# facebookresearch/FlowDec

Hardware: AMD Instinct MI355X
Metric: 48 kHz audio-seconds/sec (RTF) for FlowDec-75m @ 6 ODE steps (higher is better)
Workload: dtype bf16; 1 GPU; flowdec_75m enhance(): global batch=8 x 2 s clips @48 kHz (8 per GPU), 6-step euler (NFE 6), T_pad=256 frames, inputs resident in HBM, initial noise drawn inside the timed call, output waveforms all-gathered; global_batch=8, nfe=6, parallelism=batch-shard x1, hipgraph=True, conv_algo=auto

## Files before the change

flowdec_amd/_lib.py:

```python
import ctypes as C
import os

import torch

_HERE = os.path.dirname(os.path.abspath(__file__))
LIB_PATH = os.environ.get("FLOWDEC_HIP_LIB") or os.path.join(_HERE, "libflowdec_hip.so")

FD_F32, FD_BF16 = 0, 1
FD_WINOGRAD = 0x100
FD_WINOGRAD4 = 0x80000
FD_TILE_REVERSED = 0x100000
FD_WINOGRAD44 = 0x200000
FD_WINOGRAD_LOWRES = 0x200
FD_WINOGRAD_AUTO = 0x400
FD_LOW_LATENCY = 0x800
FD_BF16_OPERANDS = 0x10000
FD_NO_SIDE_STREAM = 0x40000
FD_EBUSY = -5
FD_BF16X3_OPERANDS = 0x20000
FD_TILE = {0: 0, 32: 0x1000, 64: 0x2000, 128: 0x3000, "64c": 0x4000, "32c": 0x5000, "duo": 0x6000, "persist": 0x7000}
CONV_KERNELS = ("DIRECT", "DIRECT_MIXED", "DIRECT_SPLIT", "WINO", "WINO4", "WINO4F", "WINO44F", "HEAD", "HEADF")
FIR_FAMILIES = ("UP", "DOWN", "DOWN_MARCH")
SOLVERS = {"euler": 0, "midpoint": 1, "heun2": 2, "heun2_eulerlast": 3}
ADAPTIVE_SOLVERS = {"dopri5": 0, "tsit5": 1}
# ... 62 lines not shown
    "fd_gn_silu_apply": (c_int, [_P, _P, _P, c_int, c_ll, c_int, c_int, _P]),
    "fd_op_pack_input": (c_int, [_P, _P, _P, c_int, c_int, c_int, c_int, _P]),
    "fd_op_combine": (c_int, [_P, _P, _P, _P, _P, _P, c_int, c_int, c_int, c_int, c_int, _P]),
    "fd_op_output_update": (c_int, [_P, _P, _P, _P, c_float, _P, _P, c_int, c_int, c_int, c_int, c_int, _P]),
    "fd_op_score_update": (c_int, [_P, _P, _P, c_float, _P, c_float, c_float, _P, _P, c_int, c_float, _P, c_int, c_int, c_int, c_int, c_int, _P]),
    "fd_op_init_state": (c_int, [_P, _P, _P, _P, c_int, _P, c_int, c_float, _P, c_int, c_int, c_int, _P]),
    "fd_op_caxpy": (c_int, [_P, _P, _P, c_int, c_float, _P, c_int, c_int, c_int, _P]),
    "fd_op_ode_lincomb": (c_int, [_P, c_float, c_float, C.POINTER(_P), C.POINTER(c_float), c_int, _P, c_ll, _P]),
    "fd_op_ode_lincomb_clips": (c_int, [_P, c_float, _P, C.POINTER(_P), C.POINTER(c_float), c_int, _P, c_int, c_ll, _P]),
    "fd_op_ode_scaled_sq": (c_int, [_P, _P, _P, _P, c_float, c_float, _P, c_int, c_ll, _P]),
    "fd_op_ode_scaled_sq_clips": (c_int, [_P, _P, _P, _P, c_float, c_float, _P, c_int, c_int, c_ll, _P]),
    "fd_op_ode_commit_clips": (c_int, [_P, _P, _P, _P, _P, _P, _P, c_int, c_ll, _P]),
    "fd_resblock_workspace_bytes": (c_size_t, [C.POINTER(FdResblockDesc), c_int, c_int, c_int, c_int]),
    "fd_resblock": (c_int, [C.POINTER(FdResblockDesc), _P, _P, _P, c_int, c_int, c_int, c_int, _P, c_size_t, _P]),
    "fd_attn_block_workspace_bytes": (c_size_t, [C.POINTER(FdAttnDesc), c_int, c_int, c_int, c_int]),
    "fd_attn_block": (c_int, [C.POINTER(FdAttnDesc), _P, _P, _P, c_int, c_int, c_int, c_int, _P, c_size_t, _P]),
    "fd_gn_finalize": (c_int, [_P, c_int, c_int, c_int, _P, c_int, c_int, c_int, _P, _P, _P, c_int, c_int, c_ll, c_float, _P]),
    "fd_conv_packed_bytes": (c_ll, [c_int] * 7),
    "fd_conv_pack_weights": (c_int, [_P, _P, _P, c_int, c_int, c_int, c_int, c_int, c_int, c_int, _P]),
    "fd_conv_cout_pad": (c_int, [c_int]),
    "fd_conv_stats_tiles": (c_int, [c_int, c_int]),
    "fd_conv2d": (c_int, [_P, c_int, _P, c_int, _P, _P, c_int, _P, c_int, _P, _P, c_int, _P, c_float, _P, c_int, _P,
                          c_int, c_int, c_int, c_int, c_int, _P]),
    "fd_conv_kernel_counts": (c_int, [C.POINTER(c_ll), c_int]),
    "fd_time_embedding": (c_int, [_P, c_int, _P, c_int, _P, _P, _P, _P, _P, _P]),
    "fd_temb_bias": (c_int, [_P, c_int, c_int, _P, _P, _P, c_int, _P, _P]),
    "fd_stft_workspace_bytes": (c_size_t, [c_int] * 4),
    "fd_stft_plan_create": (c_int, [c_int, c_int, C.POINTER(c_void_p)]),
    "fd_stft_plan_destroy": (None, [_P]),
    "fd_stft_compress": (c_int, [_P, _P, c_int, c_int, c_float, c_float, c_int, _P, _P, c_int, _P, c_size_t, _P]),
    "fd_decompress_istft": (c_int, [_P, _P, c_int, c_int, c_int, c_float, c_float, _P, _P, c_int, _P, c_size_t, _P]),
    "fd_stft_compress_ragged": (c_int, [_P, _P, _P, c_int, c_int, c_float, c_float, c_int, _P, _P, c_int, _P, c_size_t, _P]),
    "fd_decompress_istft_ragged": (c_int, [_P, _P, _P, c_int, c_int, c_int, c_float, c_float, _P, _P, c_int, _P, c_size_t, _P]),
    "fd_compress_spec": (c_int, [_P, _P, c_ll, c_float, c_float, c_int, _P]),
    "fd_stft_tables": (c_int, [c_int, c_int, _P, _P, _P]),
    "fd_stft_gemm_variant": (c_int, [c_int] * 3),
    "fd_stft_gemm_f32": (c_int, [_P, _P, _P, c_int, c_int, c_int, _P]),
    "fd_istft_envelope_ok": (c_int, [c_int] * 4),
    "fd_num_frames": (c_int, [c_int, c_int]),
    "fd_padded_frames": (c_int, [c_int]),
    "fd_model_create": (c_int, [C.POINTER(FdModelConfig), C.POINTER(_P)]),
    "fd_model_create_ex": (c_int, [C.POINTER(FdModelConfig), C.POINTER(FdModelArch), C.POINTER(_P)]),
    "fd_model_destroy": (None, [_P]),
    "fd_model_num_params": (c_int, [_P]),
    "fd_model_param_info": (c_int, [_P, c_int, C.POINTER(C.c_char_p), C.POINTER(c_int), C.POINTER(c_int * 4)]),
    "fd_model_set_param": (c_int, [_P, C.c_char_p, _P, c_ll]),
# ... 147 lines not shown
```

flowdec_amd/build.py:

```python
import os
import subprocess
import sys
from concurrent.futures import ThreadPoolExecutor

HERE = os.path.dirname(os.path.abspath(__file__))
CSRC = os.path.join(HERE, "csrc")
INC = os.path.join(os.path.dirname(HERE), "include")
LIB = os.path.join(HERE, "libflowdec_hip.so")
SOURCES = ["api.hip", "calib.hip", "conv_mfma.hip", "conv_wino.hip", "conv_wino4.hip", "conv_wino4f.hip", "conv_wino44f.hip", "conv_head.hip", "conv_headf.hip", "elementwise.hip", "ops_api.hip", "stft.hip", "metrics.hip", "estimate.hip", "loss.hip", "model.hip", "solve.hip", "enhance.hip", "attn.hip", "ndac.hip", "ndac_mfma.hip", "stream.hip", "resample.hip", "stoi.hip", "specdist.hip", "xcorr.hip"]
FLAGS = ["--offload-arch=gfx950", "-O3", "-std=c++17", "-fPIC", "-fno-slp-vectorize", "-I" + INC, "-I" + CSRC, "-Wno-unused-result"]


def _hipcc():
    for c in (os.environ.get("HIPCC"), "/opt/rocm/bin/hipcc", "hipcc"):
        if c and (os.path.isabs(c) and os.path.exists(c) or not os.path.isabs(c)):
            return c
    return "hipcc"


def needs_build():
    if not os.path.exists(LIB):
        return True
    t = os.path.getmtime(LIB)
    deps = [os.path.join(CSRC, f) for f in os.listdir(CSRC)] + [os.path.join(INC, "flowdec_hip.h"), os.path.abspath(__file__)]
    return any(os.path.getmtime(d) > t for d in deps)


def check_wino4_isa(hipcc=None, extra=()):
    import tempfile
    if os.environ.get("FLOWDEC_SKIP_ISA_CHECK", "") not in ("", "0"):
        print("flowdec_amd.build: FLOWDEC_SKIP_ISA_CHECK set -- conv_wino4.hip ISA properties NOT verified", file=sys.stderr)
        return False
# ... 56 lines not shown
```

flowdec_amd/csrc/conv_common.h:

```cpp
#pragma once
#include "common.h"
#include "internal.h"

#ifdef FD_TIMING2
#define FD_T2(...) __VA_ARGS__
#else
#define FD_T2(...)
#endif

namespace fdconv {

typedef unsigned int u32x4 __attribute__((ext_vector_type(4)));

constexpr int ROWB = 80;
constexpr int WROWB = 64;
constexpr int PITCH = 24;

struct Seg {
  const void* src;
  int C;
  int aff_off;
  int taps;
};

// ... 39 lines not shown
int fd_wino4_launch(fdconv::ConvArgs a, hipStream_t st);
int fd_wino4_init_attributes();
bool fd_wino4_supported(int Cout, int C0, int C1, int S0, int S1, int ksize);
bool fd_wino4_shape_ok(int H, int W);

long long fd_wino4f_packed_bytes(int Cout, int C0, int C1, int S0, int S1);
int fd_wino4f_pack_weights(const float* w, const float* w_sc, void* packed, int Cout, int C0, int C1, int S0, int S1, hipStream_t st);
int fd_wino4f_launch(fdconv::ConvArgs a, hipStream_t st);
int fd_wino4f_init_attributes();
bool fd_wino4f_supported(int Cout, int C0, int C1, int S0, int S1, int ksize);
bool fd_wino4f_shape_ok(int H, int W);

long long fd_wino44f_packed_bytes(int Cout, int C0, int C1, int S0, int S1);
int fd_wino44f_pack_weights(const float* w, const float* w_sc, void* packed, int Cout, int C0, int C1, int S0, int S1, hipStream_t st);
int fd_wino44f_launch(fdconv::ConvArgs a, hipStream_t st);
int fd_wino44f_init_attributes();
bool fd_wino44f_supported(int Cout, int C0, int C1, int S0, int S1, int ksize);
bool fd_wino44f_shape_ok(int H, int W);

bool fd_head_supported(const fdconv::ConvArgs& a, int ksize, int dtype);
int fd_head_launch(fdconv::ConvArgs a, hipStream_t st);
int fd_head_init_attributes();

bool fd_headf_supported(const fdconv::ConvArgs& a, int ksize, int dtype);
int fd_headf_launch(fdconv::ConvArgs a, hipStream_t st);
int fd_headf_init_attributes();
```

flowdec_amd/csrc/conv_mfma.hip:

```cpp
#include <string.h>

#include <atomic>
#include <mutex>
#include <type_traits>

#include "conv_common.h"

namespace {

using namespace fdconv;
typedef float f32x2 __attribute__((ext_vector_type(2)));

template <typename T>
struct Math;
template <>
struct Math<bf16> {
  static constexpr int EPS = 8;
  __device__ static __forceinline__ void mma(f32x16& acc, const u32x4& wf, const u32x4& pf) {
    acc = __builtin_amdgcn_mfma_f32_32x32x16_bf16(__builtin_bit_cast(bf16x8, wf), __builtin_bit_cast(bf16x8, pf), acc, 0, 0, 0);
  }
};
template <>
struct Math<float> {
  static constexpr int EPS = 4;
// ... 1161 lines not shown
  a.affine = affine; a.affC = C0 + C1;
  a.w = packed_w; a.w_bytes = fd_conv_packed_bytes(Cout, C0, C1, ksize, S0, S1, dtype | (wino ? FD_WINOGRAD : 0) | (wino4 ? FD_WINOGRAD4 : 0) | (wino44 ? FD_WINOGRAD44 : 0) | (mixed ? FD_BF16_OPERANDS : 0) | (split ? FD_BF16X3_OPERANDS : 0));
  a.bias = bias; a.bias_rows = bias_rows; a.skip = skip; a.scale = scale; a.out = out; a.Cout = Cout; a.CoutPad = cout_pad(Cout);
  a.stats = stats; a.B = B; a.H = H; a.W = W; a.reversed = reversed ? 1 : 0;
  FD_T2(a.dbg = g_dbg;)
  FD_REQUIRE(a.w_bytes < (1ll << 31), "fd_conv2d: packed weights exceed 2 GiB");
  FD_REQUIRE(affine == nullptr || (C0 + C1) * 8 <= AFF_BYTES, "fd_conv2d: at most %d activated input channels", AFF_BYTES / 8);
  if (wino44) {
    FD_REQUIRE(fd_wino44f_supported(Cout, C0, C1, S0, S1, ksize) && fd_wino44f_shape_ok(H, W),
               "fd_conv2d: FD_F32 | FD_WINOGRAD44 needs ksize 3, Cout %% 128 == 0, channel counts %% 8 == 0, H %% 16 == W %% 16 == 0");
    return counted(FD_CONV_KERNEL_WINO44F, fd_wino44f_launch(a, fd_stream(stream)));
  }
  if (wino4f) return counted(FD_CONV_KERNEL_WINO4F, fd_wino4f_launch(a, fd_stream(stream)));
  if (wino4) return counted(FD_CONV_KERNEL_WINO4, fd_wino4_launch(a, fd_stream(stream)));
  if (wino) return counted(FD_CONV_KERNEL_WINO, fd_wino_launch(a, fd_stream(stream)));
  if (mixed) return counted(FD_CONV_KERNEL_DIRECT_MIXED, dispatch_conv_mixed(a, fd_stream(stream)));
  if (split) return counted(FD_CONV_KERNEL_DIRECT_SPLIT, dispatch_conv_split(a, fd_stream(stream)));
  if (bn_hint == 0 && fd_head_supported(a, ksize, dtype)) return counted(FD_CONV_KERNEL_HEAD, fd_head_launch(a, fd_stream(stream)));
  if (bn_hint == 0 && tile == 0 && fd_headf_supported(a, ksize, dtype)) return counted(FD_CONV_KERNEL_HEADF, fd_headf_launch(a, fd_stream(stream)));
  if (dtype == FD_BF16)
    return counted(FD_CONV_KERNEL_DIRECT, dispatch_conv<bf16>(a, fd_stream(stream), bn_hint, tile == FD_TILE_BN64_CHUNK || tile == FD_TILE_BN32_CHUNK, tile == FD_TILE_PERSIST));
  return counted(FD_CONV_KERNEL_DIRECT, dispatch_conv<float>(a, fd_stream(stream), bn_hint, false));
}
```

flowdec_amd/csrc/internal.h:

```cpp
#pragma once
#include "common.h"

struct fd_temb_job {
  const float* dense_w;
  const float* dense_b;
  const float* conv_b;
  float* out;
  int Cout;
};

struct fd_noise_src {
  const float* ptr = nullptr;
  const unsigned long long* seeds = nullptr;
  int draw = 0;
  const int* frame0 = nullptr;
};

struct fd_edge_args {
  const void* x = nullptr;
  const void* y = nullptr;
  const float* w = nullptr;
  const float* bias = nullptr;
  void* out = nullptr;
  const void* base = nullptr;
// ... 5 lines not shown
  float cb = 1.f, cy = 0.f, cz = 0.f;
  int B = 0, H = 0, W = 0, Cout = 0;
  int ks = 1;
};

int fd_time_embedding_impl(const float* t, float t_imm, int nt, const float* gfp_w, int nf, const float* w1, const float* b1,
                           const float* w2, const float* b2, float* temb, hipStream_t st);
int fd_temb_bias_batched(const fd_temb_job* jobs_dev, int njobs, const float* temb, int nt, int temb_dim, hipStream_t st);
int fd_edge_op(int which, const fd_edge_args& a, int dtype, hipStream_t st);
int fd_init_state(const float* Y, const fd_noise_src& noise, const double* sigma_dev, int sigma_n, float sigma_fac, float* x0, int B,
                  int F, int T, hipStream_t st);
int fd_combine_tiles(int H, int W);
int fd_ode_lincomb(const float* x, float cx, float dt, const float* const* k, const float* c, int nk, float* dst, long long n, hipStream_t st);
int fd_ode_scaled_sq(const float* p, const float* q, const float* r, const float* s, float atol, float rtol, double* partial, int nblocks,
                     long long n, hipStream_t st);
int fd_ode_lincomb_clips(const float* x, float cx, const float* dt_dev, const float* const* k, const float* c, int nk, float* dst, int B, long long n,
                         hipStream_t st);
int fd_ode_scaled_sq_clips(const float* p, const float* q, const float* r, const float* s, float atol, float rtol, double* partial, int nblocks, int B,
                           long long n, hipStream_t st);
int fd_ode_commit_clips(const int* accept, const int* ckpt, const float* x_new, const float* k6, float* x, float* k0, float* traj, int B, long long n,
                        hipStream_t st);
int fd_caxpy(const float* a, const fd_noise_src& q, float cq, float* dst, int B, int F, int T, hipStream_t st);
int fd_conv_init_attributes();
int fd_stft_forward(fd_stft_plan* p, const float* y, const int* lens, int B, int L, float alpha, float beta, int normalize, float* normfac,
                    float* Y, int T_pad, void* ws, size_t ws_bytes, hipStream_t st, const float* normfac_in = nullptr);
int fd_stft_inverse(fd_stft_plan* p, const float* X, const int* lens, int B, int T, int T_pad, float alpha, float beta, const float* normfac,
                    float* y, int L, void* ws, size_t ws_bytes, hipStream_t st);
size_t fd_stft_ws_bytes(int B, int L, int n_fft, int hop);
void fd_stft_plan_dims(const fd_stft_plan* p, int* n_fft, int* hop, int* n_freq, int* kpad);
int fd_stft_kpad(int n_fft);
int fd_stft_raw_spectrum(fd_stft_plan* p, const float* y, const int* lens, int B, int L, float* frames, float* spec, hipStream_t st);
void fd_resample_plan_dims(const fd_resample_plan* p, int* o, int* n, int* width, int* K);
bool fd_ndac_mfma_supported(int Ci, int Co, int K, int stride, int dil, int transposed);
void fd_ndac_mfma_pack(const float* w_ci_k_co, int Ci, int Co, int K, int stride, int transposed, void* dst);
int fd_ndac_mfma_conv(const float* x, const void* wp, const float* bias, const float* res, float* out, float* out_act, const float* alpha_out, int B,
                      int Ci, int T, int Co, int K, int stride, int pad, int dil, int transposed, hipStream_t st);
void fd_ndac_weight_ci_k_co(const float* w, int Ci, int Co, int K, int transposed, float* dst);
size_t fd_attn_qkv_bytes(int B, int N, int C);
int fd_attn_stats_tiles(int H, int W);
int fd_attn_launch(const void* x, const float* affine, const fd_attn_desc& d, float* qkv, void* out, float* stats, int B, int N, int dtype,
                   hipStream_t st);
```

flowdec_amd/csrc/model.hip:

```cpp
#include <string>
#include <vector>

#include "arena.h"
#include "model_internal.h"

using namespace fdm;

namespace {

struct Tens {
  size_t off = (size_t)-1;
  int C = 0, H = 0, W = 0;
  size_t sums = (size_t)-1;
  int tiles = 0, stride = 0;
};

int gn_groups(int C) { return (C / 4 < 32) ? C / 4 : 32; }

void build_structure(fd_model* m) {
  const fd_model_config& c = m->cfg;
  const int nf = c.nf, R = c.num_levels, nrb = c.num_res_blocks, nch = 4;
  auto& mods = m->mods;
  auto& P = m->params;
  mods.clear(); P.clear();
// ... 70 lines not shown
  FD_HIP(hipMemcpy(d, it->second.data(), sizeof(float) * it->second.size(), hipMemcpyHostToDevice));
  m->dev_allocs.push_back(d);
  m->dev_f32[name] = d;
  *out = d;
  return FD_OK;
}

int pack_conv(fd_model* m, const std::string& name, int Cout, int C0, int C1, const std::string& sc_name, int S0, int S1, int algo,
              const void** out, hipStream_t st) {
  float *src = nullptr, *sc = nullptr;
  FD_TRY(upload_f32(m, name, &src));
  if (!sc_name.empty()) FD_TRY(upload_f32(m, sc_name, &sc));
  void* dst = nullptr;
  const int wdtype = m->dt | algo | m->opflag;
  const long long bytes = fd_conv_packed_bytes(Cout, C0, C1, 3, S0, S1, wdtype);
  FD_REQUIRE(bytes > 0, "internal: no packing for conv '%s'", name.c_str());
  FD_HIP(hipMalloc(&dst, (size_t)bytes));
  m->dev_allocs.push_back(dst);
  FD_TRY(fd_conv_pack_weights(src, sc, dst, Cout, C0, C1, 3, S0, S1, wdtype, st));
  *out = dst;
  return FD_OK;
}

int pack_rb_conv(fd_model* m, int level, const std::string& name, int Cout, int C0, int C1, const std::string& sc_name, int S0, int S1,
                 ConvW* w, hipStream_t st) {
  auto fits = [&](int algo) { return fd_conv_packed_bytes(Cout, C0, C1, 3, S0, S1, m->dt | algo) > 0; };
  auto pack = [&](int algo, const void** out) { return pack_conv(m, name, Cout, C0, C1, sc_name, S0, S1, algo, out, st); };
  const bool f23_only = m->sched == CS_WINOGRAD || (m->sched == CS_WINOGRAD_LOWRES && level >= 2);
  if (f23_only && fits(FD_WINOGRAD)) return pack(FD_WINOGRAD, &w->f23);
  const bool by_size = m->sched == CS_AUTO || m->sched == CS_LATENCY;
  if (by_size && fits(FD_WINOGRAD)) FD_TRY(pack(FD_WINOGRAD, &w->f23));
  if (by_size && fits(FD_WINOGRAD4)) FD_TRY(pack(FD_WINOGRAD4, &w->f43));
  if (m->sched == CS_AUTO_F32 && fits(FD_WINOGRAD44)) FD_TRY(pack(FD_WINOGRAD44, &w->f44));
  return pack(0, &w->direct);
}

struct ConvPick { const void* w; int flags; };
ConvPick pick_conv(ConvSchedule s, const ConvW& w, int px_tiles, bool whole_tiles, int cin, int cout, bool shortcut) {
  const bool autosel = s == CS_AUTO, latency = s == CS_LATENCY;
  if (s == CS_AUTO_F32 && w.f44 && whole_tiles) return {w.f44, FD_WINOGRAD44};
  if (latency && px_tiles <= 24 && cout >= 64) return {w.direct, FD_TILE_BN32_CHUNK};
  if (autosel && px_tiles <= 16 && cout >= 64) return {w.direct, FD_TILE_BN64_CHUNK};
  if ((autosel || latency) && w.f23 && !shortcut && px_tiles <= (latency ? 128 : 96)) return {w.f23, FD_WINOGRAD};
  if ((autosel || (latency && px_tiles > 128)) && w.f43 && whole_tiles && cin >= 64) return {w.f43, FD_WINOGRAD4};
  if (latency && px_tiles <= 128 && cout >= 256 && cout % 128 == 0) return {w.direct, FD_TILE_BN128};
  return w.direct ? ConvPick{w.direct, 0} : ConvPick{w.f23, FD_WINOGRAD};
// ... 77 lines not shown
    int flags = pick.flags;
    if (flags == FD_WINOGRAD4 && !dry && (w4_launches++ & 1) != 0) flags |= FD_TILE_REVERSED;
    if (want_stats) {
      out.tiles = fd_conv_stats_tiles(out.H, out.W);
      out.stride = fd_conv_cout_pad(out.C);
      out.sums = arena.alloc(sizeof(float) * 2 * (size_t)B * out.tiles * out.stride);
    }
    if (dry) return FD_OK;
    const bool prof = m && m->profiling;
    auto launch = [&]() {
      return fd_conv2d(ptr(a.off), a.C, b ? ptr(b->off) : nullptr, b ? b->C : 0, aff == (size_t)-1 ? nullptr : (const float*)ptr(aff),
                       s0 ? ptr(s0->off) : nullptr, s0 ? s0->C : 0, s1 ? ptr(s1->off) : nullptr, s1 ? s1->C : 0, pick.w, bias, bias_rows,
                       skip ? ptr(skip->off) : nullptr, scale, ptr(out.off), out.C, want_stats ? (float*)ptr(out.sums) : nullptr, B,
                       out.H, out.W, ks, dt | flags | (m ? m->opflag : 0), st);
    };
    const int rc = prof ? timed(m->ev, m->ev_used, launch) : launch();
    if (prof) {
      const double csc = (s0 ? s0->C : 0) + (s1 ? s1->C : 0);
      m->prof_flops += 2.0 * B * out.H * out.W * (double)out.C * (cin * ks * ks + csc);
      const double exec = (flags & FD_WINOGRAD44) ? 0.25 : (flags & FD_WINOGRAD4) ? 0.5 : (flags & FD_WINOGRAD) ? 2.0 / 3.0 : 1.0;
      m->prof_flops_exec += 2.0 * B * out.H * out.W * (double)out.C * (cin * ks * ks * exec + csc);
      m->prof_bytes += (double)B * out.H * out.W * esz * (cin + csc + (skip ? out.C : 0) + out.C) + (double)esz * out.C * (cin * ks * ks + csc);
    }
    return rc;
  }

  int fir(const void* x, const float* aff, void* o_raw, void* o_act, int H, int W, int C, int dir) {
    const bool prof = m && m->profiling;
    auto launch = [&]() { return fd_fir_resample(x, aff, o_raw, o_act, B, H, W, C, dir, dt, st); };
    const int rc = prof ? timed(m->ev_fir, m->ev_fir_used, launch) : launch();
    if (prof) {
      const double in = (double)B * H * W * C * esz, out1 = dir > 0 ? 4.0 * in : 0.25 * in;
      m->prof_fir_bytes += in + out1 * ((o_raw ? 1 : 0) + (o_act ? 1 : 0));
    }
    return rc;
  }

  int resblock(const Mod& md, Tens& x0, Tens* x1, int nt, Tens& out, bool out_given = false) {
    const float rs2 = 0.70710678118654752440f;
    size_t aff0;
    FD_TRY(gn_affine(x0, x1, md.gn0_g, md.gn0_b, &aff0));
    const int H = x0.H, W = x0.W;
    const int OH = md.up ? 2 * H : (md.down ? H / 2 : H), OW = md.up ? 2 * W : (md.down ? W / 2 : W);
    Tens h1 = talloc(md.cout, OH, OW);
    Tens xr, hr;
    if (md.up || md.down) {
// ... 110 lines not shown
      }
      FD_TRY(resblock(mods[mi++], a1, nullptr, nt, a2));
      tfree(a1);
      h = a2;
    }
    Tens pyramid; bool have_pyr = false;
    for (int lvl = R - 1; lvl >= 0; --lvl) {
      for (int b = 0; b < nrb + 1; ++b) {
        Tens sk = hs.back(); hs.pop_back();
        Tens o;
        FD_TRY(resblock(mods[mi++], h, &sk, nt, o));
        tfree(h); tfree(sk);
        h = o;
      }
      const Mod& gn = mods[mi++];
      const Mod& head = mods[mi++];
      if (side) FD_TRY(fork());
      size_t aff;
      FD_TRY(gn_affine(h, nullptr, gn.gn0_g, gn.gn0_b, &aff));
      Tens pnew = talloc(4, h.H, h.W);
      if (have_pyr) {
        Tens pu = talloc(4, h.H, h.W);
        if (!dry) FD_TRY(fir(ptr(pyramid.off), nullptr, ptr(pu.off), nullptr, pyramid.H, pyramid.W, 4, +1));
        FD_TRY(conv(h, nullptr, aff, nullptr, nullptr, head.conv0, head.b_f32, 1, &pu, 1.f, pnew, false));
        release_later(pu.off, side); release_later(pyramid.off, side);
        pu.off = pyramid.off = (size_t)-1;
      } else {
        FD_TRY(conv(h, nullptr, aff, nullptr, nullptr, head.conv0, head.b_f32, 1, nullptr, 1.f, pnew, false));
      }
      release_later(aff, side);
      pyramid = pnew; have_pyr = true;
      if (side) back();
      if (lvl != 0) {
        Tens o;
        FD_TRY(resblock(mods[mi++], h, nullptr, nt, o));
        if (side) FD_TRY(join());
        tfree(h);
        h = o;
      } else if (side) {
        FD_TRY(join());
      }
    }
    tfree(h);
    if (!hs.empty() || mi != mods.size()) return fd_set_error(FD_ESTATE, "internal: module walk mismatch");
    if (!dry) {
      fd_edge_args a; a.x = ptr(pyramid.off); a.w = m->wo; a.base = os.base; a.kold = os.kold; a.coef = os.coef; a.out = os.dst; a.ksave = os.ksave;
      a.B = B; a.H = F; a.W = T; a.ks = m->arch.output_ksize;
      if (os.score) { a.y = os.yv; a.z = os.z; a.cb = os.cb; a.cy = os.cy; a.cz = os.cz; }
      FD_TRY(fd_edge_op(os.score ? 4 : 3, a, dt, st));
    }
    tfree(pyramid);
// ... 185 lines not shown
      case M_ATTN: {
        FD_TRY(upload_f32(m, p + "GroupNorm_0.weight", &md.gn0_g)); FD_TRY(upload_f32(m, p + "GroupNorm_0.bias", &md.gn0_b));
        const int Cc = md.cout;
        std::vector<float>& wq = m->host[p + "qkv.W"];
        std::vector<float>& bq = m->host[p + "qkv.b"];
        wq.assign((size_t)Cc * 3 * Cc, 0.f); bq.assign((size_t)3 * Cc, 0.f);
        for (int k = 0; k < 3; ++k) {
          const std::vector<float>& w = m->host[p + "NIN_" + std::to_string(k) + ".W"];
          const std::vector<float>& bb = m->host[p + "NIN_" + std::to_string(k) + ".b"];
          for (int r = 0; r < Cc; ++r)
            for (int c = 0; c < Cc; ++c) wq[(size_t)r * 3 * Cc + k * Cc + c] = w[(size_t)r * Cc + c];
          for (int c = 0; c < Cc; ++c) bq[(size_t)k * Cc + c] = bb[c];
        }
        FD_TRY(upload_f32(m, p + "qkv.W", &md.w_qkv)); FD_TRY(upload_f32(m, p + "qkv.b", &md.b_qkv));
        FD_TRY(upload_f32(m, p + "NIN_3.W", &md.w_f32)); FD_TRY(upload_f32(m, p + "NIN_3.b", &md.b_f32));
        break;
      }
      case M_GN:
        FD_TRY(upload_f32(m, p + "weight", &md.gn0_g));
        FD_TRY(upload_f32(m, p + "bias", &md.gn0_b));
        break;
      case M_CONV_HEAD:
        FD_TRY(pack_conv(m, p + "weight", md.cout, md.cin, 0, "", 0, 0, 0, &md.conv0.direct, st));
        FD_TRY(upload_f32(m, p + "bias", &md.b_f32));
        break;
      case M_RB: {
        FD_TRY(upload_f32(m, p + "GroupNorm_0.weight", &md.gn0_g)); FD_TRY(upload_f32(m, p + "GroupNorm_0.bias", &md.gn0_b));
        FD_TRY(upload_f32(m, p + "GroupNorm_1.weight", &md.gn1_g)); FD_TRY(upload_f32(m, p + "GroupNorm_1.bias", &md.gn1_b));
        FD_TRY(pack_rb_conv(m, md.level, p + "Conv_0.weight", md.cout, md.c0, md.c1, "", 0, 0, &md.conv0, st));
        FD_TRY(pack_rb_conv(m, md.level, p + "Conv_1.weight", md.cout, md.cout, 0, md.has_c2 ? p + "Conv_2.weight" : std::string(),
                            md.has_c2 ? md.c0 : 0, md.has_c2 ? md.c1 : 0, &md.conv1, st));
        if (md.has_c2) {
          std::vector<float>& b1 = m->host[p + "Conv_1.bias"];
          const std::vector<float>& b2 = m->host[p + "Conv_2.bias"];
          for (size_t i = 0; i < b1.size(); ++i) b1[i] += b2[i];
        }
        FD_TRY(upload_f32(m, p + "Conv_1.bias", &md.b1));
        fd_temb_job j{};
        FD_TRY(upload_f32(m, p + "Dense_0.weight", &tmp)); j.dense_w = tmp;
        FD_TRY(upload_f32(m, p + "Dense_0.bias", &tmp)); j.dense_b = tmp;
        FD_TRY(upload_f32(m, p + "Conv_0.bias", &tmp)); j.conv_b = tmp;
        md.bias0_eff = bias_pool + bias_off; bias_off += (size_t)fd_model::MAX_NT * md.cout;
        j.out = md.bias0_eff; j.Cout = md.cout;
        jobs.push_back(j);
        break;
      }
// ... 151 lines not shown
```

flowdec_amd/csrc/model_internal.h:

```cpp
#pragma once
#include <atomic>
#include <map>
#include <set>
#include <string>
#include <tuple>
#include <vector>

#include "common.h"
#include "internal.h"

namespace fdm {

enum ModKind { M_GFP, M_LINEAR, M_CONV_IN, M_RB, M_COMBINE, M_GN, M_CONV_HEAD, M_ATTN };

enum ConvSchedule { CS_DIRECT, CS_WINOGRAD, CS_WINOGRAD_LOWRES, CS_AUTO, CS_LATENCY, CS_AUTO_F32 };

struct ConvW { const void *direct = nullptr, *f23 = nullptr, *f43 = nullptr, *f44 = nullptr; };

struct Mod {
  ModKind kind;
  int idx;
  int cin = 0, cout = 0;
  int c0 = 0, c1 = 0;
  bool up = false, down = false, has_c2 = false;
  int level = 0;
  ConvW conv0, conv1;
  float *gn0_g = nullptr, *gn0_b = nullptr, *gn1_g = nullptr, *gn1_b = nullptr;
  float* b1 = nullptr;
  float* bias0_eff = nullptr;
  float *w_f32 = nullptr, *b_f32 = nullptr;
  float *w_qkv = nullptr, *b_qkv = nullptr;
};

struct ParamInfo {
  std::string name;
  std::vector<int> shape;
  long long numel() const { long long n = 1; for (int s : shape) n *= s; return n; }
};

struct GraphKey {
// ... 122 lines not shown
```

flowdec_amd/ops.py:

```python
import math

import torch

from . import _lib as L


def _nhwc(x):
    L.require_cuda(x)
    if x.ndim != 4 or not x.is_contiguous():
        raise RuntimeError("expected a contiguous NHWC tensor [B, H, W, C]")
    return x.shape


def to_nhwc(x_nchw, dtype=None):
    return x_nchw.permute(0, 2, 3, 1).contiguous().to(dtype or x_nchw.dtype)


def to_nchw(x_nhwc):
    return x_nhwc.permute(0, 3, 1, 2).contiguous()


def channel_sums(x):
    B, H, W, Cc = _nhwc(x)
    tiles = L.load().fd_channel_sums_tiles(H, W)
# ... 66 lines not shown
    nbytes = L.load().fd_conv_packed_bytes(Cout, C0, Cin - C0, k, S0, S - S0, dt)
    if nbytes <= 0:
        raise RuntimeError("flowdec_hip: this convolution shape has no %s packing" % ("Winograd" if winograd else "MFMA"))
    packed = torch.empty(nbytes, dtype=torch.uint8, device=w.device)
    L.check(L.load().fd_conv_pack_weights(L.ptr(w), L.ptr(w_sc), L.ptr(packed), Cout, C0, Cin - C0, k, S0, S - S0, dt, L.stream()))
    return packed


def conv2d(x0, packed_w, Cout, ksize, x1=None, affine=None, bias=None, skip=None, scale=1.0, sc0=None, sc1=None, want_stats=False,
           winograd=False, tile_bn=0, bf16_operands=False, reversed_tiles=False):
    B, H, W, C0 = _nhwc(x0)
    lib = L.load()
    C1 = 0 if x1 is None else x1.shape[3]
    S0 = 0 if sc0 is None else sc0.shape[3]
    S1 = 0 if sc1 is None else sc1.shape[3]
    out = torch.empty(B, H, W, Cout, dtype=x0.dtype, device=x0.device)
    stats = torch.zeros(B, lib.fd_conv_stats_tiles(H, W), lib.fd_conv_cout_pad(Cout), 2, dtype=torch.float32, device=x0.device) if want_stats else None
    rows = 0 if bias is None else (1 if bias.ndim == 1 else bias.shape[0])
    L.check(lib.fd_conv2d(L.ptr(x0), C0, L.ptr(x1), C1, L.ptr(affine), L.ptr(sc0), S0, L.ptr(sc1), S1, L.ptr(packed_w), L.ptr(bias), rows,
                          L.ptr(skip), float(scale), L.ptr(out), Cout, L.ptr(stats), B, H, W, ksize,
                          L.dtype_id(x0.dtype) | _WINO[winograd] | (L.FD_TILE_REVERSED if reversed_tiles else 0) | L.FD_TILE[tile_bn] | {False: 0, True: L.FD_BF16_OPERANDS, "x3": L.FD_BF16X3_OPERANDS}[bf16_operands],
                          L.stream()))
    return (out, stats) if want_stats else out


def conv_kernel_counts():
    import ctypes as C
    n = len(L.CONV_KERNELS)
    buf = (C.c_longlong * n)()
    total = L.load().fd_conv_kernel_counts(buf, n)
    if total != n:
        raise RuntimeError(f"flowdec_hip: fd_conv_kernel_counts reports {total} kernel families, the binding knows {n}")
    return dict(zip(L.CONV_KERNELS, buf))


def ndac_mfma_pack_weights(w, stride=1, transposed=False):
    import numpy as np
    w = np.ascontiguousarray(w, dtype=np.float32)
    Ci, Co = (w.shape[0], w.shape[1]) if transposed else (w.shape[1], w.shape[0])
    K = w.shape[2]
    nb = L.load().fd_ndac_mfma_packed_bytes(Ci, Co, K, stride, int(transposed))
    out = np.zeros(max(nb, 2) // 2, np.uint16)
    L.check(L.load().fd_ndac_mfma_pack_weights(w.ctypes.data, Ci, Co, K, stride, int(transposed), out.ctypes.data))
    return out


# ... 303 lines not shown
```

include/flowdec_hip.h:

```cpp
#ifndef FLOWDEC_HIP_H
#define FLOWDEC_HIP_H

#include <stddef.h>
#include <stdint.h>

#ifdef __cplusplus
extern "C" {
#endif

#define FD_OK 0
#define FD_EINVAL (-1)
#define FD_ERUNTIME (-2)
#define FD_ENOMEM (-3)
#define FD_ESTATE (-4)
#define FD_EBUSY (-5)

#define FD_F32 0
#define FD_BF16 1
#define FD_WINOGRAD 0x100
#define FD_WINOGRAD4 0x80000
#define FD_WINOGRAD44 0x200000
#define FD_TILE_REVERSED 0x100000
#define FD_WINOGRAD_LOWRES 0x200
#define FD_WINOGRAD_AUTO 0x400
// ... 35 lines not shown
#define FD_FIR_UP 0
#define FD_FIR_DOWN 1
#define FD_FIR_DOWN_MARCH 2
int fd_fir_variant(int B, int H, int W, int C, int direction, int dtype, int has_affine, int want_raw, int want_act);

int fd_conv_in(const void* in8, const float* w, const float* bias, void* out, float* stats, int B, int H, int W, int Cout, int dtype,
               void* stream);

int fd_channel_sums_tiles(int H, int W);
int fd_channel_sums(const void* x, float* part, int B, int H, int W, int C, int dtype, void* stream);
int fd_gn_finalize(const float* part0, int tiles0, int stride0, int C0, const float* part1, int tiles1, int stride1, int C1,
                   const float* gamma, const float* beta, float* affine, int B, int groups, long long hw, float eps,
                   void* stream);

long long fd_conv_packed_bytes(int Cout, int C0, int C1, int ksize, int S0, int S1, int wdtype);
int fd_conv_pack_weights(const float* w, const float* w_sc, void* packed, int Cout, int C0, int C1, int ksize, int S0, int S1,
                         int wdtype, void* stream);
int fd_conv_cout_pad(int Cout);
int fd_conv_stats_tiles(int H, int W);

int fd_conv2d(const void* in0, int C0, const void* in1, int C1, const float* affine, const void* sc0, int S0, const void* sc1,
              int S1, const void* packed_w, const float* bias, int bias_rows, const void* skip, float scale, void* out,
              int Cout, float* stats, int B, int H, int W, int ksize, int dtype, void* stream);

enum { FD_CONV_KERNEL_DIRECT, FD_CONV_KERNEL_DIRECT_MIXED, FD_CONV_KERNEL_DIRECT_SPLIT, FD_CONV_KERNEL_WINO,
       FD_CONV_KERNEL_WINO4, FD_CONV_KERNEL_WINO4F, FD_CONV_KERNEL_WINO44F, FD_CONV_KERNEL_HEAD,
       FD_CONV_KERNEL_HEADF, FD_CONV_KERNEL_COUNT };
int fd_conv_kernel_counts(long long* counts, int n);

int fd_time_embedding(const float* t, int nt, const float* gfp_w, int nf, const float* w1, const float* b1,
                      const float* w2, const float* b2, float* temb, void* stream);
int fd_temb_bias(const float* temb, int nt, int temb_dim, const float* dense_w, const float* dense_b,
                 const float* conv_bias, int Cout, float* out, void* stream);

int fd_gn_silu_apply(const void* x, const float* affine, void* out, int B, long long hw, int C, int dtype, void* stream);

typedef struct fd_resblock_desc {
  int cin0, cin1, cout, up, down, has_conv2;
  const float *gn0_gamma, *gn0_beta, *gn1_gamma, *gn1_beta;
  const void* w0; const float* bias0; int bias0_rows;
  const void* w1; const float* bias1;
} fd_resblock_desc;
size_t fd_resblock_workspace_bytes(const fd_resblock_desc* d, int B, int H, int W, int dtype);
int fd_resblock(const fd_resblock_desc* d, const void* x0, const void* x1, void* out, int B, int H, int W, int dtype, void* ws,
                size_t ws_bytes, void* stream);

// ... 287 lines not shown
```

Before: 133.6 audio-seconds/second.

## Add two-pass per-tap MFMA head conv for Cout=4 output heads

Adds a new head convolution path for 3x3 convs with four output channels and at least 128 input channels. The first kernel applies the GroupNorm affine and SiLU inline, then computes all nine tap products per pixel as one bf16 MFMA GEMM into an fp32 workspace. The second kernel gathers the shifted tap results and adds bias and skip. This aims to avoid the poor MFMA utilisation of a generic direct conv with tiny Cout, in exchange for an extra kernel launch and a 144-byte-per-pixel workspace round trip through memory.

```diff
diff --git a/flowdec_amd/_lib.py b/flowdec_amd/_lib.py
--- a/flowdec_amd/_lib.py
+++ b/flowdec_amd/_lib.py
@@ -108,6 +108,12 @@
     "fd_conv_stats_tiles": (c_int, [c_int, c_int]),
     "fd_conv2d": (c_int, [_P, c_int, _P, c_int, _P, _P, c_int, _P, c_int, _P, _P, c_int, _P, c_float, _P, c_int, _P,
                           c_int, c_int, c_int, c_int, c_int, _P]),
+    "fd_head2_packed_bytes": (c_ll, [c_int]),
+    "fd_head2_pack_weights": (c_int, [_P, _P, c_int, _P]),
+    "fd_head2_ws_bytes": (c_size_t, [c_int, c_int, c_int]),
+    "fd_head2_launch_count": (c_ll, []),
+    "fd_conv2d_head_ws": (c_int, [_P, c_int, _P, c_int, _P, _P, _P, _P, c_int, _P, c_float, _P, c_int, c_int, c_int, c_int, c_int, c_int,
+                                  _P, c_size_t, _P]),
     "fd_conv_kernel_counts": (c_int, [C.POINTER(c_ll), c_int]),
     "fd_time_embedding": (c_int, [_P, c_int, _P, c_int, _P, _P, _P, _P, _P, _P]),
     "fd_temb_bias": (c_int, [_P, c_int, c_int, _P, _P, _P, c_int, _P, _P]),
diff --git a/flowdec_amd/build.py b/flowdec_amd/build.py
--- a/flowdec_amd/build.py
+++ b/flowdec_amd/build.py
@@ -7,7 +7,7 @@
 CSRC = os.path.join(HERE, "csrc")
 INC = os.path.join(os.path.dirname(HERE), "include")
 LIB = os.path.join(HERE, "libflowdec_hip.so")
-SOURCES = ["api.hip", "calib.hip", "conv_mfma.hip", "conv_wino.hip", "conv_wino4.hip", "conv_wino4f.hip", "conv_wino44f.hip", "conv_head.hip", "conv_headf.hip", "elementwise.hip", "ops_api.hip", "stft.hip", "metrics.hip", "estimate.hip", "loss.hip", "model.hip", "solve.hip", "enhance.hip", "attn.hip", "ndac.hip", "ndac_mfma.hip", "stream.hip", "resample.hip", "stoi.hip", "specdist.hip", "xcorr.hip"]
+SOURCES = ["api.hip", "calib.hip", "conv_mfma.hip", "conv_wino.hip", "conv_wino4.hip", "conv_wino4f.hip", "conv_wino44f.hip", "conv_head.hip", "conv_head2.hip", "conv_headf.hip", "elementwise.hip", "ops_api.hip", "stft.hip", "metrics.hip", "estimate.hip", "loss.hip", "model.hip", "solve.hip", "enhance.hip", "attn.hip", "ndac.hip", "ndac_mfma.hip", "stream.hip", "resample.hip", "stoi.hip", "specdist.hip", "xcorr.hip"]
 FLAGS = ["--offload-arch=gfx950", "-O3", "-std=c++17", "-fPIC", "-fno-slp-vectorize", "-I" + INC, "-I" + CSRC, "-Wno-unused-result"]
 
 
diff --git a/flowdec_amd/csrc/conv_common.h b/flowdec_amd/csrc/conv_common.h
--- a/flowdec_amd/csrc/conv_common.h
+++ b/flowdec_amd/csrc/conv_common.h
@@ -85,6 +85,9 @@
 int fd_head_launch(fdconv::ConvArgs a, hipStream_t st);
 int fd_head_init_attributes();
 
+int fd_head2_launch(const void* in0, int C, const float* affine, const void* packed_taps, const float* bias, int bias_rows, const void* skip,
+                    float scale, void* out, int B, int H, int W, void* ws, hipStream_t st);
+
 bool fd_headf_supported(const fdconv::ConvArgs& a, int ksize, int dtype);
 int fd_headf_launch(fdconv::ConvArgs a, hipStream_t st);
 int fd_headf_init_attributes();
diff --git a/flowdec_amd/csrc/conv_head2.hip b/flowdec_amd/csrc/conv_head2.hip
--- /dev/null
+++ b/flowdec_amd/csrc/conv_head2.hip
@@ -0,0 +1,214 @@
+#include <atomic>
+
+#include "conv_common.h"
+
+namespace {
+
+using namespace fdconv;
+
+constexpr int NTH = 256;
+constexpr int TAPB = 144;
+constexpr int MAX_BPW = 16;
+
+struct TapArgs {
+  const void* x; int C;
+  const float* affine;
+  const void* w;
+  float* T;
+  int HW, nblk16, bpw, wg_per_img;
+};
+
+struct GatherArgs {
+  const float* T;
+  const float* bias; int bias_rows;
+  const void* skip;
+  float scale;
+  void* out;
+  int H, W, wg_per_img;
+};
+
+__device__ __forceinline__ u32x4 act_slot(u32x4 raw, const char* ad) {
+  u32x4 out;
+#pragma unroll
+  for (int j = 0; j < 4; ++j) {
+    const f32x4 a = *reinterpret_cast<const f32x4*>(ad + 16 * j);
+    const unsigned u = raw[j];
+    const float x0 = __builtin_bit_cast(float, u << 16), x1 = __builtin_bit_cast(float, u & 0xffff0000u);
+    bf16x2 r = {(bf16)fd_silu(fmaf(x0, a[0], a[1])), (bf16)fd_silu(fmaf(x1, a[2], a[3]))};
+    out[j] = __builtin_bit_cast(unsigned, r);
+  }
+  return out;
+}
+
+template <int NK, bool ACT>
+__global__ __launch_bounds__(NTH) void head_taps_kernel(TapArgs p) {
+  __shared__ __attribute__((aligned(16))) char afftab[ACT ? NK * 32 * 8 : 16];
+  const int t = threadIdx.x, lane = t & 63, wave = t >> 6;
+  const int b = blockIdx.x / p.wg_per_img, wg = blockIdx.x - b * p.wg_per_img;
+  constexpr int C = NK * 32;
+  if constexpr (ACT) {
+    const float* ap = p.affine + (size_t)b * C * 2;
+    for (int i = t; i < C / 2; i += NTH) *reinterpret_cast<f32x4*>(afftab + i * 16) = *reinterpret_cast<const f32x4*>(ap + i * 4);
+  }
+  u32x4 wf[NK][3];
+#pragma unroll
+  for (int ks = 0; ks < NK; ++ks)
+#pragma unroll
+    for (int rb = 0; rb < 3; ++rb) wf[ks][rb] = *reinterpret_cast<const u32x4*>(reinterpret_cast<const char*>(p.w) + ((ks * 3 + rb) * 64 + lane) * 16);
+  if constexpr (ACT) __syncthreads();
+
+  const int blk0 = (wg * 4 + wave) * p.bpw;
+  if (blk0 >= p.nblk16) return;
+  const int nb = p.nblk16 - blk0 < p.bpw ? p.nblk16 - blk0 : p.bpw;
+  const int px0 = blk0 * 16;
+  const int npx = p.HW - px0 < nb * 16 ? p.HW - px0 : nb * 16;
+  const size_t pix = (size_t)b * p.HW + px0;
+  const __amdgpu_buffer_rsrc_t srd = band_rsrc(reinterpret_cast<const bf16*>(p.x) + pix * C, (unsigned)npx * C * (unsigned)sizeof(bf16));
+  const int col = lane & 15, kg = lane >> 4;
+  const int loff = col * C * 2 + kg * 16;
+  char* tp[3];
+#pragma unroll
+  for (int rb = 0; rb < 3; ++rb)
+    tp[rb] = reinterpret_cast<char*>(p.T) + (((size_t)b * 9 + (rb < 2 ? 4 * rb + kg : 8)) * p.HW + px0 + col) * 16;
+
+  auto load = [&](u32x4 (&r)[NK], int blk) {
+#pragma unroll
+    for (int ks = 0; ks < NK; ++ks) r[ks] = __builtin_amdgcn_raw_buffer_load_b128(srd, loff + blk * (16 * C * 2) + ks * 64, 0, 0);
+  };
+  auto consume = [&](u32x4 (&r)[NK], int blk) {
+    if constexpr (ACT) asm volatile("" ::: "memory");
+    f32x4 acc[3] = {{0.f, 0.f, 0.f, 0.f}, {0.f, 0.f, 0.f, 0.f}, {0.f, 0.f, 0.f, 0.f}};
+#pragma unroll
+    for (int ks = 0; ks < NK; ++ks) {
+      u32x4 v = r[ks];
+      if constexpr (ACT) v = act_slot(v, afftab + (ks * 32 + kg * 8) * 8);
+#pragma unroll
+      for (int rb = 0; rb < 3; ++rb)
+        acc[rb] = __builtin_amdgcn_mfma_f32_16x16x32_bf16(__builtin_bit_cast(bf16x8, wf[ks][rb]), __builtin_bit_cast(bf16x8, v), acc[rb], 0, 0, 0);
+    }
+    if (blk * 16 + col < npx) {
+      *reinterpret_cast<f32x4*>(tp[0] + blk * 256) = acc[0];
+      *reinterpret_cast<f32x4*>(tp[1] + blk * 256) = acc[1];
+      if (kg == 0) *reinterpret_cast<f32x4*>(tp[2] + blk * 256) = acc[2];
+    }
+  };
+  u32x4 ra[NK], rb_[NK];
+  load(ra, 0);
+  for (int blk = 0; blk < nb; blk += 2) {
+    if (blk + 1 < nb) load(rb_, blk + 1);
+    consume(ra, blk);
+    if (blk + 1 < nb) {
+      if (blk + 2 < nb) load(ra, blk + 2);
+      consume(rb_, blk + 1);
+    }
+  }
+}
+
+template <bool SKIP>
+__global__ __launch_bounds__(NTH) void head_gather_kernel(GatherArgs p) {
+  const int b = blockIdx.x / p.wg_per_img, p0 = (blockIdx.x - b * p.wg_per_img) * NTH;
+  const int t = threadIdx.x;
+  const int H = p.H, W = p.W, HW = H * W;
+  const int px = p0 + t;
+  if (px >= HW) return;
+  const int h = px / W, w = px - h * W;
+  f32x4 v = {0.f, 0.f, 0.f, 0.f};
+#pragma unroll
+  for (int tap = 0; tap < 9; ++tap) {
+    const char* const tb = reinterpret_cast<const char*>(p.T) + (((size_t)b * 9 + tap) * HW + p0) * 16;
+    const int dh = tap / 3 - 1, dw = tap % 3 - 1;
+    if (h + dh >= 0 && h + dh < H && w + dw >= 0 && w + dw < W) {
+      const f32x4 q = *reinterpret_cast<const f32x4*>(tb + (t + dh * W + dw) * 16);
+#pragma unroll
+      for (int j = 0; j < 4; ++j) v[j] += q[j];
+    }
+  }
+  const size_t o = ((size_t)b * HW + px) * 4;
+  if constexpr (SKIP) {
+    const bf16x4 s = *reinterpret_cast<const bf16x4*>(reinterpret_cast<const bf16*>(p.skip) + o);
+#pragma unroll
+    for (int j = 0; j < 4; ++j) v[j] += (float)s[j];
+  }
+  float bv[4] = {0.f, 0.f, 0.f, 0.f};
+  if (p.bias) {
+    const float* bp = p.bias + (size_t)(p.bias_rows > 1 ? b : 0) * 4;
+#pragma unroll
+    for (int j = 0; j < 4; ++j) bv[j] = bp[j];
+  }
+  bf16x4 r;
+#pragma unroll
+  for (int j = 0; j < 4; ++j) r[j] = (bf16)((v[j] + bv[j]) * p.scale);
+  *reinterpret_cast<bf16x4*>(reinterpret_cast<bf16*>(p.out) + o) = r;
+}
+
+__global__ void head2_pack_kernel(const float* w, bf16* packed, int C) {
+  const int i = blockIdx.x * blockDim.x + threadIdx.x;
+  if (i >= C * 48) return;
+  const int j = i & 7, lane = (i >> 3) & 63, rb = (i >> 9) % 3, ks = (i >> 9) / 3;
+  const int row = rb * 16 + (lane & 15), c = ks * 32 + 8 * (lane >> 4) + j;
+  const int tap = row >> 2, o = row & 3;
+  packed[i] = row < 36 ? (bf16)w[((size_t)o * C + c) * 9 + tap] : (bf16)0.f;
+}
+
+template <int NK>
+void launch_taps(const TapArgs& a, bool act, dim3 grid, hipStream_t st) {
+  if (act) hipLaunchKernelGGL((head_taps_kernel<NK, true>), grid, dim3(NTH), 0, st, a);
+  else hipLaunchKernelGGL((head_taps_kernel<NK, false>), grid, dim3(NTH), 0, st, a);
+}
+
+std::atomic<long long> g_head2_launches{0};
+
+}
+
+bool fd_head2_supported(int C0, int C1, int Cout, int ksize, int dtype) {
+  return dtype == FD_BF16 && ksize == 3 && Cout == 4 && C1 == 0 && C0 > 0 && C0 % 32 == 0 && C0 <= 256;
+}
+
+extern "C" long long fd_head2_packed_bytes(int C) { return C > 0 && C % 32 == 0 && C <= 256 ? (long long)C * 48 * 2 : 0; }
+
+extern "C" int fd_head2_pack_weights(const float* w, void* packed, int C, void* stream) {
+  FD_REQUIRE(w && packed, "fd_head2_pack_weights: null pointer");
+  FD_REQUIRE(fd_head2_packed_bytes(C) > 0, "fd_head2_pack_weights: C must be a multiple of 32, at most 256 (got %d)", C);
+  hipLaunchKernelGGL(head2_pack_kernel, dim3(fd_cdiv(C * 48, 256)), dim3(256), 0, fd_stream(stream), w, reinterpret_cast<bf16*>(packed), C);
+  FD_LAUNCH_CHECK();
+  return FD_OK;
+}
+
+extern "C" size_t fd_head2_ws_bytes(int B, int H, int W) { return (size_t)B * H * W * TAPB; }
+
+extern "C" long long fd_head2_launch_count() { return g_head2_launches.load(std::memory_order_relaxed); }
+
+int fd_head2_launch(const void* in0, int C, const float* affine, const void* packed_taps, const float* bias, int bias_rows, const void* skip,
+                    float scale, void* out, int B, int H, int W, void* ws, hipStream_t st) {
+  const long long HW = (long long)H * W;
+  TapArgs a{};
+  a.x = in0; a.C = C; a.affine = affine; a.w = packed_taps; a.T = reinterpret_cast<float*>(ws);
+  a.HW = (int)HW; a.nblk16 = fd_cdiv(HW, 16);
+  a.bpw = a.nblk16 / (4 * 64) < 1 ? 1 : a.nblk16 / (4 * 64) > MAX_BPW ? MAX_BPW : a.nblk16 / (4 * 64);
+  a.wg_per_img = fd_cdiv(a.nblk16, 4 * a.bpw);
+  const long long nblk = (long long)B * a.wg_per_img;
+  GatherArgs g{};
+  g.T = a.T; g.bias = bias; g.bias_rows = bias_rows; g.skip = skip; g.scale = scale; g.out = out; g.H = H; g.W = W;
+  g.wg_per_img = fd_cdiv(HW, NTH);
+  const long long gblk = (long long)B * g.wg_per_img;
+  FD_REQUIRE(nblk > 0 && nblk < (1ll << 31) && gblk < (1ll << 31), "conv grid out of range");
+  FD_REQUIRE(W < (1 << 26), "fd_conv2d_head_ws: W = %d exceeds 2^26 pixels (32-bit neighbour offsets of the gather)", W);
+  const dim3 grid((unsigned)nblk);
+  switch (C / 32) {
+    case 1: launch_taps<1>(a, affine != nullptr, grid, st); break;
+    case 2: launch_taps<2>(a, affine != nullptr, grid, st); break;
+    case 3: launch_taps<3>(a, affine != nullptr, grid, st); break;
+    case 4: launch_taps<4>(a, affine != nullptr, grid, st); break;
+    case 5: launch_taps<5>(a, affine != nullptr, grid, st); break;
+    case 6: launch_taps<6>(a, affine != nullptr, grid, st); break;
+    case 7: launch_taps<7>(a, affine != nullptr, grid, st); break;
+    case 8: launch_taps<8>(a, affine != nullptr, grid, st); break;
+    default: return fd_set_error(FD_EINVAL, "fd_conv2d_head_ws: internal: %d channels", C);
+  }
+  FD_LAUNCH_CHECK();
+  if (skip) hipLaunchKernelGGL((head_gather_kernel<true>), dim3((unsigned)gblk), dim3(NTH), 0, st, g);
+  else hipLaunchKernelGGL((head_gather_kernel<false>), dim3((unsigned)gblk), dim3(NTH), 0, st, g);
+  FD_LAUNCH_CHECK();
+  g_head2_launches.fetch_add(1, std::memory_order_relaxed);
+  return FD_OK;
+}
diff --git a/flowdec_amd/csrc/conv_mfma.hip b/flowdec_amd/csrc/conv_mfma.hip
--- a/flowdec_amd/csrc/conv_mfma.hip
+++ b/flowdec_amd/csrc/conv_mfma.hip
@@ -1207,3 +1207,16 @@
     return counted(FD_CONV_KERNEL_DIRECT, dispatch_conv<bf16>(a, fd_stream(stream), bn_hint, tile == FD_TILE_BN64_CHUNK || tile == FD_TILE_BN32_CHUNK, tile == FD_TILE_PERSIST));
   return counted(FD_CONV_KERNEL_DIRECT, dispatch_conv<float>(a, fd_stream(stream), bn_hint, false));
 }
+
+extern "C" int fd_conv2d_head_ws(const void* in0, int C0, const void* in1, int C1, const float* affine, const void* packed_w,
+                                 const void* packed_taps, const float* bias, int bias_rows, const void* skip, float scale, void* out, int Cout,
+                                 int B, int H, int W, int ksize, int dtype, void* ws, size_t ws_bytes, void* stream) {
+  if (!(packed_taps && ws && in1 == nullptr && fd_head2_supported(C0, C1, Cout, ksize, dtype)))
+    return fd_conv2d(in0, C0, in1, C1, affine, nullptr, 0, nullptr, 0, packed_w, bias, bias_rows, skip, scale, out, Cout, nullptr, B, H, W, ksize, dtype, stream);
+  FD_REQUIRE(in0 && out, "fd_conv2d_head_ws: null pointer");
+  FD_REQUIRE(B > 0 && H > 0 && W > 0, "fd_conv2d_head_ws: bad shape");
+  FD_REQUIRE(bias == nullptr || bias_rows == 1 || bias_rows == B, "fd_conv2d_head_ws: bias_rows must be 1 or B");
+  FD_REQUIRE((long long)H * W < (1ll << 31), "fd_conv2d_head_ws: an image of %d x %d pixels exceeds 2^31 pixels (32-bit pixel indices)", H, W);
+  FD_REQUIRE(ws_bytes >= fd_head2_ws_bytes(B, H, W), "fd_conv2d_head_ws: workspace %zu < required %zu bytes", ws_bytes, fd_head2_ws_bytes(B, H, W));
+  return counted(FD_CONV_KERNEL_HEAD, fd_head2_launch(in0, C0, affine, packed_taps, bias, bias_rows, skip, scale, out, B, H, W, ws, fd_stream(stream)));
+}
diff --git a/flowdec_amd/csrc/internal.h b/flowdec_amd/csrc/internal.h
--- a/flowdec_amd/csrc/internal.h
+++ b/flowdec_amd/csrc/internal.h
@@ -51,6 +51,7 @@
                         hipStream_t st);
 int fd_caxpy(const float* a, const fd_noise_src& q, float cq, float* dst, int B, int F, int T, hipStream_t st);
 int fd_conv_init_attributes();
+bool fd_head2_supported(int C0, int C1, int Cout, int ksize, int dtype);
 int fd_stft_forward(fd_stft_plan* p, const float* y, const int* lens, int B, int L, float alpha, float beta, int normalize, float* normfac,
                     float* Y, int T_pad, void* ws, size_t ws_bytes, hipStream_t st, const float* normfac_in = nullptr);
 int fd_stft_inverse(fd_stft_plan* p, const float* X, const int* lens, int B, int T, int T_pad, float alpha, float beta, const float* normfac,
diff --git a/flowdec_amd/csrc/model.hip b/flowdec_amd/csrc/model.hip
--- a/flowdec_amd/csrc/model.hip
+++ b/flowdec_amd/csrc/model.hip
@@ -116,6 +116,8 @@
   return FD_OK;
 }
 
+constexpr int HEAD2_MIN_C = 128;
+
 int pack_rb_conv(fd_model* m, int level, const std::string& name, int Cout, int C0, int C1, const std::string& sc_name, int S0, int S1,
                  ConvW* w, hipStream_t st) {
   auto fits = [&](int algo) { return fd_conv_packed_bytes(Cout, C0, C1, 3, S0, S1, m->dt | algo) > 0; };
@@ -239,6 +241,28 @@
       m->prof_flops_exec += 2.0 * B * out.H * out.W * (double)out.C * (cin * ks * ks * exec + csc);
       m->prof_bytes += (double)B * out.H * out.W * esz * (cin + csc + (skip ? out.C : 0) + out.C) + (double)esz * out.C * (cin * ks * ks + csc);
     }
+    return rc;
+  }
+
+  int head_conv(const Tens& a, size_t aff, const ConvW& w, const float* bias, const Tens* skip, Tens& out, bool on_side) {
+    if (!(w.taps && aff != (size_t)-1 && fd_head2_supported(a.C, 0, out.C, 3, dt | (m ? m->opflag : 0))))
+      return conv(a, nullptr, aff, nullptr, nullptr, w, bias, 1, skip, 1.f, out, false);
+    const size_t wsb = fd_head2_ws_bytes(B, out.H, out.W), T = arena.alloc(wsb);
+    int rc = FD_OK;
+    if (!dry) {
+      const bool prof = m && m->profiling;
+      auto launch = [&]() {
+        return fd_conv2d_head_ws(ptr(a.off), a.C, nullptr, 0, (const float*)ptr(aff), w.direct, w.taps, bias, 1, skip ? ptr(skip->off) : nullptr,
+                                 1.f, ptr(out.off), out.C, B, out.H, out.W, 3, dt | (m ? m->opflag : 0), ptr(T), wsb, st);
+      };
+      rc = prof ? timed(m->ev, m->ev_used, launch) : launch();
+      if (prof) {
+        const double fl = 2.0 * B * out.H * out.W * (double)out.C * a.C * 9;
+        m->prof_flops += fl; m->prof_flops_exec += fl;
+        m->prof_bytes += (double)B * out.H * out.W * esz * (a.C + (skip ? out.C : 0) + out.C) + (double)esz * out.C * a.C * 9;
+      }
+    }
+    release_later(T, on_side);
     return rc;
   }
 
@@ -395,11 +419,11 @@
       if (have_pyr) {
         Tens pu = talloc(4, h.H, h.W);
         if (!dry) FD_TRY(fir(ptr(pyramid.off), nullptr, ptr(pu.off), nullptr, pyramid.H, pyramid.W, 4, +1));
-        FD_TRY(conv(h, nullptr, aff, nullptr, nullptr, head.conv0, head.b_f32, 1, &pu, 1.f, pnew, false));
+        FD_TRY(head_conv(h, aff, head.conv0, head.b_f32, &pu, pnew, side));
         release_later(pu.off, side); release_later(pyramid.off, side);
         pu.off = pyramid.off = (size_t)-1;
       } else {
-        FD_TRY(conv(h, nullptr, aff, nullptr, nullptr, head.conv0, head.b_f32, 1, nullptr, 1.f, pnew, false));
+        FD_TRY(head_conv(h, aff, head.conv0, head.b_f32, nullptr, pnew, side));
       }
       release_later(aff, side);
       pyramid = pnew; have_pyr = true;
@@ -631,6 +655,13 @@
         break;
       case M_CONV_HEAD:
         FD_TRY(pack_conv(m, p + "weight", md.cout, md.cin, 0, "", 0, 0, 0, &md.conv0.direct, st));
+        if (md.cin >= HEAD2_MIN_C && fd_head2_supported(md.cin, 0, md.cout, 3, m->dt | m->opflag)) {
+          void* tp = nullptr;
+          FD_HIP(hipMalloc(&tp, (size_t)fd_head2_packed_bytes(md.cin)));
+          m->dev_allocs.push_back(tp);
+          FD_TRY(fd_head2_pack_weights(m->dev_f32[p + "weight"], tp, md.cin, st));
+          md.conv0.taps = tp;
+        }
         FD_TRY(upload_f32(m, p + "bias", &md.b_f32));
         break;
       case M_RB: {
diff --git a/flowdec_amd/csrc/model_internal.h b/flowdec_amd/csrc/model_internal.h
--- a/flowdec_amd/csrc/model_internal.h
+++ b/flowdec_amd/csrc/model_internal.h
@@ -15,7 +15,7 @@
 
 enum ConvSchedule { CS_DIRECT, CS_WINOGRAD, CS_WINOGRAD_LOWRES, CS_AUTO, CS_LATENCY, CS_AUTO_F32 };
 
-struct ConvW { const void *direct = nullptr, *f23 = nullptr, *f43 = nullptr, *f44 = nullptr; };
+struct ConvW { const void *direct = nullptr, *f23 = nullptr, *f43 = nullptr, *f44 = nullptr, *taps = nullptr; };
 
 struct Mod {
   ModKind kind;
diff --git a/flowdec_amd/ops.py b/flowdec_amd/ops.py
--- a/flowdec_amd/ops.py
+++ b/flowdec_amd/ops.py
@@ -112,6 +112,34 @@
                           L.dtype_id(x0.dtype) | _WINO[winograd] | (L.FD_TILE_REVERSED if reversed_tiles else 0) | L.FD_TILE[tile_bn] | {False: 0, True: L.FD_BF16_OPERANDS, "x3": L.FD_BF16X3_OPERANDS}[bf16_operands],
                           L.stream()))
     return (out, stats) if want_stats else out
+
+
+def pack_head_taps(w):
+    L.require_cuda(w)
+    w = w.contiguous().float()
+    nbytes = L.load().fd_head2_packed_bytes(w.shape[1]) if tuple(w.shape[2:]) == (3, 3) and w.shape[0] == 4 else 0
+    if nbytes <= 0:
+        return None
+    packed = torch.empty(nbytes, dtype=torch.uint8, device=w.device)
+    L.check(L.load().fd_head2_pack_weights(L.ptr(w), L.ptr(packed), w.shape[1], L.stream()))
+    return packed
+
+
+def conv2d_head(x0, packed_w, packed_taps, x1=None, affine=None, bias=None, skip=None, scale=1.0):
+    B, H, W, C0 = _nhwc(x0)
+    lib = L.load()
+    C1 = 0 if x1 is None else x1.shape[3]
+    out = torch.empty(B, H, W, 4, dtype=x0.dtype, device=x0.device)
+    nws = lib.fd_head2_ws_bytes(B, H, W)
+    ws = torch.empty(nws, dtype=torch.uint8, device=x0.device)
+    rows = 0 if bias is None else (1 if bias.ndim == 1 else bias.shape[0])
+    L.check(lib.fd_conv2d_head_ws(L.ptr(x0), C0, L.ptr(x1), C1, L.ptr(affine), L.ptr(packed_w), L.ptr(packed_taps), L.ptr(bias), rows,
+                                  L.ptr(skip), float(scale), L.ptr(out), 4, B, H, W, 3, L.dtype_id(x0.dtype), L.ptr(ws), nws, L.stream()))
+    return out
+
+
+def head2_launch_count():
+    return int(L.load().fd_head2_launch_count())
 
 
 def conv_kernel_counts():
diff --git a/include/flowdec_hip.h b/include/flowdec_hip.h
--- a/include/flowdec_hip.h
+++ b/include/flowdec_hip.h
@@ -81,6 +81,14 @@
 int fd_conv2d(const void* in0, int C0, const void* in1, int C1, const float* affine, const void* sc0, int S0, const void* sc1,
               int S1, const void* packed_w, const float* bias, int bias_rows, const void* skip, float scale, void* out,
               int Cout, float* stats, int B, int H, int W, int ksize, int dtype, void* stream);
+
+long long fd_head2_packed_bytes(int C);
+int fd_head2_pack_weights(const float* w, void* packed, int C, void* stream);
+size_t fd_head2_ws_bytes(int B, int H, int W);
+long long fd_head2_launch_count(void);
+int fd_conv2d_head_ws(const void* in0, int C0, const void* in1, int C1, const float* affine, const void* packed_w,
+                      const void* packed_taps, const float* bias, int bias_rows, const void* skip, float scale, void* out, int Cout,
+                      int B, int H, int W, int ksize, int dtype, void* ws, size_t ws_bytes, void* stream);
 
 enum { FD_CONV_KERNEL_DIRECT, FD_CONV_KERNEL_DIRECT_MIXED, FD_CONV_KERNEL_DIRECT_SPLIT, FD_CONV_KERNEL_WINO,
        FD_CONV_KERNEL_WINO4, FD_CONV_KERNEL_WINO4F, FD_CONV_KERNEL_WINO44F, FD_CONV_KERNEL_HEAD,
```

New measurement: 134.8 audio-seconds/second, median of 6. About the same (+0.9%).
